# pigimonaco/Pinocchio

Hardware: AMD Instinct MI355X
Metric: grid-cells/sec for full Fmax sweep (all smoothing radii) + 3LPT, 1024^3 box (higher is better)
Workload: dtype f64

## Files before the change

### pinocchio_amd/csrc/pf_api.hip

```cpp
#include <hip/hip_runtime.h>

#include <math.h>
#include <stdarg.h>
#include <stdio.h>
#include <stdlib.h>
#include <string.h>

#include <atomic>
#include <string>
#include <functional>
#include <vector>

#include "../../include/pinfmax.h"
#include "pf_collapse_core.h"
#include "pf_hostpool.h"
#include "pf_internal.h"

extern "C" void pf_rccl_release(void *link);
extern "C" int pf_rccl_link_count(void *link);

static thread_local char g_err[512] = "";
int pf_fail(int task, const char *fmt, ...) {
  va_list ap;
  va_start(ap, fmt);
// ... 102 lines not shown
  int gt_n[4];
  double gt_logkmin[4], gt_dlogk[4], gt_sign[4];
  double *gtab;
  int tab_ns;
  double tab_var[PF_MAX_SMOOTH];
  bool tab_ready;
  int tab_ismooth;
  int model;
  double sng_cosmo[7], sng_Din[PF_MAX_SMOOTH], sng_size[PF_MAX_SMOOTH];
  int sng_ns;
  PfCtDev ct;
  double *ct_block;
  bool have_density, have_hessian, have_sources, products_init;
  int sources_order;
  bool sweep_sources, sources_fresh;
  bool transposed;
  int ct_flavour;
  int lpt_order;
  double *partials_src;
  bool general;
  void *W;
  void *fft_c2r, *fft_r2c;
  bool vel_zero_pending;
  int last_ns;
  struct PfHandoff *handoff;
  PfLoopback *loopback;
  pf_alltoall_fn a2a; void *a2a_user;
  pf_alltoallv_fn a2av; void *a2av_user;
  pf_allreduce_fn ared; void *ared_user;
  void *rccl;
// ... 107 lines not shown
  t->zpass_inv_wg_per_cu = env_int("PF_ZPASS_INV_WG_PER_CU", 32);
  if (t->zpass_inv_wg_per_cu <= 0) t->zpass_inv_wg_per_cu = 32;
  t->spline_lut = env_int("PF_SPLINE_LUT", 1) != 0;
  t->exchange_rows = env_int("PF_EXCHANGE_ROWS", 1) != 0;
  t->invariants = env_int("PF_INVARIANTS", 1);
  t->lpt_fuse = env_int("PF_LPT_FUSE", 1);
  t->collapse_wg_per_cu = env_int("PF_COLLAPSE_WG_PER_CU", 8);
  if (t->collapse_wg_per_cu <= 0) t->collapse_wg_per_cu = 8;
  t->general = env_int("PF_GENERAL", 0) != 0;

  t->pipeline = env_int("PF_PIPELINE", 1) != 0;
  t->replicate = env_int("PF_REPLICATE_DK", -1);
  t->exact_libm = env_int("PF_EXACT_LIBM", 0) != 0;
  t->solve_beside_z = env_int("PF_SOLVE_BESIDE_Z", -1);
  t->gtab = env_int("PF_GTAB", 1) != 0;
  t->preflight = env_int("PF_PREFLIGHT", 1) != 0;
  t->handoff_chunk_mb = env_int("PF_HANDOFF_CHUNK_MB", 256);
  if (t->handoff_chunk_mb <= 0) t->handoff_chunk_mb = 256;
  t->handoff_threads = env_int("PF_HANDOFF_THREADS", 0);
  t->host_register = env_int("PF_HOST_REGISTER", 0) != 0;
  t->distribute_lds = env_int("PF_DISTRIBUTE_LDS", 1) != 0;
  const char *fault = getenv("PF_DEBUG_PIPELINE_FAULT");
  t->debug_fault = !fault ? 0 : !strcmp(fault, "recv") ? 1 : !strcmp(fault, "send") ? 2 : 0;
  t->prune_eps = 8.673617379884035e-19;
  if (const char *e = getenv("PF_PRUNE_EPS")) t->prune_eps = atof(e);
}

static void plan_bytes(const pf_ctx *c, size_t *at_create, size_t *peak) {
  const size_t field = c->field_bytes, nc = ncell_of(c);
  size_t fields = 1 + 3 + 6 + 3;
// ... 131 lines not shown
  if ((cfg->flags & PF_FLAG_DOUBLE_PRODUCTS) && cfg->field_bytes != 8)
    return pf_fail(rank, "pf_create: PF_FLAG_DOUBLE_PRODUCTS (fp64 Fmax and displacements) needs fp64 fields");
  int ndev = 0;
  if (hipGetDeviceCount(&ndev) != hipSuccess || ndev <= 0)
    return pf_fail(rank, "pf_create: no HIP device available (libpinfmax_hip has no CPU path)");
  if (cfg->device < 0 || cfg->device >= ndev) return pf_fail(rank, "pf_create: device %d out of range (%d devices)", cfg->device, ndev);
  pf_ctx *c = new pf_ctx();
  c->cfg = *cfg; c->rank = rank; c->P = cfg->nranks; c->n = (int)n; c->nzh = c->n / 2 + 1; c->nzp = c->n / 2 + 64 / cfg->field_bytes;
  c->tune = tune; c->dev = cfg->device; c->inv_reruns = 0;
  c->general = want_general; c->fft_c2r = c->fft_r2c = nullptr; c->W = nullptr;
  if (c->general) c->nzp = c->nzh;
  c->nxl = c->n / c->P; c->nyl = c->n / c->P; c->fb = cfg->field_bytes; c->timing = (cfg->flags & PF_FLAG_TIMING) != 0; c->pb = (cfg->flags & PF_FLAG_DOUBLE_PRODUCTS) ? 8 : 4;
  c->dev_bytes = 0; c->own_stream = true; c->stream = nullptr;
  c->a2a = nullptr; c->a2av = nullptr; c->a2av_user = nullptr; c->ared = nullptr; c->a2a_user = c->ared_user = nullptr; c->rccl = nullptr;
  c->have_density = c->have_hessian = c->have_sources = c->products_init = false; c->last_ns = 0;
  c->sweep_sources = c->sources_fresh = false; c->partials_src = nullptr; c->lpt_order = 3; c->ct_flavour = 0; c->transposed = false;
  c->vel_zero_pending = false; c->have_genic = false;
  memset(c->ks_ms, 0, sizeof(c->ks_ms)); memset(c->ks_bytes, 0, sizeof(c->ks_bytes)); memset(c->ks_n, 0, sizeof(c->ks_n));
  memset(&c->cpu, 0, sizeof(c->cpu)); memset(c->spl_set, 0, sizeof(c->spl_set)); memset(c->spl_n, 0, sizeof(c->spl_n));
  c->growth[0] = 1.0; c->growth[1] = 3. / 7.; c->growth[2] = -1. / 9.; c->growth[3] = 5. / 42.;
  for (int i = 0; i < 6; i++) { c->B[i] = nullptr; c->B2[i] = nullptr; }
  c->blockA = nullptr; c->dk = nullptr; c->recvA = nullptr; c->tw = nullptr;
  c->blockA2 = nullptr; c->recvA2 = nullptr; c->cstream = nullptr; c->dk_full = nullptr; c->replicate = false; c->dk_full_valid = false; for (int k = 0; k < 3; k++) c->INV[0][k] = c->INV[1][k] = nullptr; c->inv_w = 0; c->inv_own[0] = c->inv_own[1] = nullptr; c->blockS = c->blockB2 = nullptr;
  c->fmax = nullptr; c->rmax = nullptr; c->vel12 = nullptr; c->partials = nullptr; c->scal = nullptr; c->hist = nullptr; c->spl = nullptr;
  c->gtab = nullptr; c->etab = nullptr; c->ct_block = nullptr; c->gt = nullptr; c->gt_lut = nullptr;
  memset(c->gt_ok, 0, sizeof(c->gt_ok)); memset(c->gt_err, 0, sizeof(c->gt_err));
  for (int i = 0; i < 2; i++) c->ev_x[i] = c->ev_r[i] = c->ev_y[i] = c->ev_s[i] = nullptr;
  c->sstream = nullptr; c->solve_ran_beside = false; c->loopback = nullptr; c->handoff = nullptr;
  c->pipeline = c->P > 1 && tune.pipeline;
  for (int i = 0; i < 3; i++) { c->A[i] = nullptr; c->S[i] = nullptr; }
  memset(c->gt_n, 0, sizeof(c->gt_n));
// ... 232 lines not shown
  PfAddr a; a.os = c->nzp; a.el_shift = ilog2i(c->n); a.el_len = c->n; a.ehs = 0; a.els = (long long)c->n * c->nzp; return a;
}
static PfAddr addr_local_x(const pf_ctx *c, int zp) {
  PfAddr a; a.os = (long long)c->nxl * zp; a.el_shift = ilog2i(c->nxl); a.el_len = c->nxl; a.ehs = 0; a.els = zp; return a;
}
static PfAddr addr_local_y(const pf_ctx *c, int zp) {
  PfAddr a; a.os = zp; a.el_shift = ilog2i(c->n); a.el_len = c->n; a.ehs = 0; a.els = (long long)c->nxl * zp; return a;
}
static PfAddr addr_xs_y(const pf_ctx *c) {
  PfAddr a; a.os = (long long)c->n * c->nzp; a.el_shift = ilog2i(c->n); a.el_len = c->n; a.ehs = 0; a.els = c->nzp; return a;
}

struct Job { const void *in; void *out; int mul; };

static int xpass(pf_ctx *c, int kind, int dir, int njobs, const Job *jobs, int pre, double rs, double growth, int nin, int band = 1 << 30,
                 bool out_yblocks = false, bool replicated = false) {
  PfStridedParams p; memset(&p, 0, sizeof(p));
  p.njobs = njobs;
  for (int j = 0; j < njobs; j++) { p.job[j].in = jobs[j].in; p.job[j].out = jobs[j].out; p.job[j].mul = jobs[j].mul; }
  p.ain = p.aout = addr_ky_x(c);
  if (out_yblocks) p.aout = addr_yblocks_x(c, band_zpitch(c, band));
  p.ncols = c->nzh; p.nouter = c->nyl; p.pre = pre; p.outer_offset = c->rank * c->nyl; p.rs = rs; p.growth = growth; p.tw = c->tw;
  p.etab = c->etab; p.dev = c->dev;
  if (replicated) {
    p.ain = addr_full_x(c); p.aout = addr_local_x(c, band_zpitch(c, band));
    p.nouter = c->n; p.outer_offset = 0; p.out_e0 = c->rank * c->nxl; p.out_ne = c->nxl;
  }
  if (pre && rs != 0.0) PFCHK(c, pf_launch_exp_table(c->etab, c->n, rs, c->stream));
  p.band_e = p.band_outer = c->n;
  double frac_cols = 1.0, frac_in = 1.0, frac_outer = 1.0;
  if (band < c->n / 2) {
    p.band_e = p.band_outer = band;
    p.ncols = band + 1;
    frac_cols = (double)(band + 1) / c->nzh; frac_in = frac_outer = (double)(2 * band + 1) / c->n;
  }
  KTimer t(c, kind, (nin * frac_in * (replicated ? c->P : 1) + njobs) * frac_cols * frac_outer * spec_bytes_alg(c));
  PFCHK(c, pf_launch_strided(c->fb, c->n, dir, p, c->stream));
  return 0;
}
static int ypass(pf_ctx *c, int kind, int dir, int njobs, const Job *jobs, bool in_blocks, bool out_blocks, int nin, int band = 1 << 30,
                 bool in_yblocks = false, bool in_local = false) {
  PfStridedParams p; memset(&p, 0, sizeof(p));
  p.njobs = njobs;
  for (int j = 0; j < njobs; j++) { p.job[j].in = jobs[j].in; p.job[j].out = jobs[j].out; p.job[j].mul = jobs[j].mul; }
  p.ain = in_blocks ? (in_yblocks ? addr_yblocks_y(c, band_zpitch(c, band)) : addr_blocks_y(c)) : addr_xs_y(c);
  if (in_local) p.ain = addr_local_y(c, band_zpitch(c, band));
  p.aout = out_blocks ? addr_blocks_y(c) : addr_xs_y(c);
  p.ncols = c->nzh; p.nouter = c->nxl; p.pre = 0; p.outer_offset = 0; p.rs = 0; p.growth = 1; p.tw = c->tw; p.dev = c->dev;
  p.band_e = p.band_outer = c->n;
  double frac_cols = 1.0, frac_in = 1.0;
  if (band < c->n / 2) {
// ... 12 lines not shown
  p.njobs = njobs;
  double outb = 0;
  for (int j = 0; j < njobs; j++) {
    p.job[j].in = jobs[j].in; p.job[j].out = jobs[j].out; p.job[j].mul = jobs[j].mul; p.job[j].out_f32 = jobs[j].f32;
    outb += jobs[j].f32 ? (double)ncell(c) * 4.0 : real_bytes_alg(c);
  }
  p.nlines = (long long)c->nxl * c->n; p.in_pitch = c->nzp; p.out_pitch = 2 * c->nzp;
  p.norm = 1.0 / ((double)c->n * c->n * c->n); p.dc = dc; p.tw = c->tw;
  p.band_k = c->n;
  double frac_in = 1.0;
  if (band < c->n / 2) { p.band_k = band; frac_in = (double)(band + 1) / c->nzh; }
  p.ncu = c->ncu; p.dev = c->dev; p.persist_per_cu = c->tune.zpass_persist; p.inv_per_cu = c->tune.zpass_inv_wg_per_cu;
  p.flag = c->scal + SC_INV_FLAG;
  if (acc) {
    p.acc = acc;
    KTimer t(c, KS_ZPASS_LPT3B, njobs * frac_in * spec_bytes_alg(c) + 8.0 * real_bytes_alg(c));
    PFCHK(c, pf_launch_c2r_invariants(c->fb, c->n, p, c->stream, 1));
    return 0;
  }
  if (invariants) {
    if (c->fb == 4) {
      if (inv_rows(c, c->inv_w)) return 1;
      for (int k = 0; k < 3; k++) p.inv_out[k] = c->INV[c->inv_w][k];
      p.inv_pitch = c->n;
      if (c->inv_w == 0) c->have_sources = false;
    }
    KTimer t(c, KS_ZPASS_INV, njobs * frac_in * spec_bytes_alg(c) + 3.0 * (double)ncell(c) * 8.0);
    PFCHK(c, pf_launch_c2r_invariants(c->fb, c->n, p, c->stream));
    return 0;
  }
  KTimer t(c, kind, njobs * frac_in * spec_bytes_alg(c) + outb);
  PFCHK(c, pf_launch_c2r(c->fb, c->n, p, c->stream));
// ... 92 lines not shown
      PFCHK(c, g_c2r(c, c->W, tmp));
      PFCHK(c, pf_launch_real_to_col((const double *)tmp, velcol(c, 3 * orders[j] + ia - 1), nc, c->pb, c->stream));
    }
  return 0;
}
static int g_forward_of(pf_ctx *c, void *f) {
  PFCHK(c, g_r2c(c, f, c->W));
  HIPCHK(c, hipMemcpyAsync(f, c->W, c->field_bytes, hipMemcpyDeviceToDevice, c->stream));
  return 0;
}
static int g_reverse_of(pf_ctx *c, void *f) {
  PFCHK(c, g_filter(c, f, c->W, -1, -1, 0.0, 0, true));
  return g_c2r(c, c->W, f);
}

static int hess_band(const pf_ctx *c, double rs) {
  int band = 1 << 30;
  if (rs > 0.0 && c->prune_eps > 0.0) {
    const double kc = sqrt(-2.0 * log(c->prune_eps)) / rs;
    const double kb = kc * c->n / (2.0 * 3.14159265358979323846);
    if (kb < c->n / 2 - 1) band = (int)kb + 1;
  }
  return band;
}
static int hess_x(pf_ctx *c, const void *spec, double rs, void *const A[3], int band, bool replicated = false) {
  const Job xj[3] = {{spec, A[0], PF_MUL_ONE}, {spec, A[1], PF_MUL_K}, {spec, A[2], PF_MUL_K2}};
  return xpass(c, KS_XPASS_HESS, +1, 3, xj, 1, rs, 1.0, 1, band, true, replicated);
}
static int ensure_dk_full(pf_ctx *c) {
  if (!c->replicate || c->dk_full_valid) return 0;
  if (c->a2a == loopback_a2a && c->have_genic) {
    unsigned int *dseed = nullptr;
    const int rc = pf_genic_launch(c->fb, c->dk_full, c->n, c->nzp, c->n, 0, &c->genic, c->stream, &dseed);
    if (!rc) HIPCHK(c, hipStreamSynchronize(c->stream));
    hipFree(dseed);
    if (rc) return pf_fail(c->rank, "pf_genic_density (whole spectrum): launch failed");
    c->dk_full_valid = true;
    return 0;
  }
  const size_t rows = (size_t)c->nyl * c->nzp * 2 * c->fb;
  HIPCHK(c, hipMemsetAsync(c->dk_full, 0, (size_t)c->P * c->field_bytes, c->stream));
  HIPCHK(c, hipMemcpy2DAsync((char *)c->dk_full + (size_t)c->rank * rows, (size_t)c->P * rows, c->dk, rows, rows, (size_t)c->n,
// ... 28 lines not shown
  return pipelined_band(c, 1, 3,
                        [&](int, void *const *A) { return hess_x(c, rep ? c->dk_full : spec, rs, A, band, rep); },
                        [&](int, int set, int f) { return recv_field(c, set, f); },
                        [&](int, const void *const *R) { return hess_yz(c, R, dc, out, band, false, acc, hfirst, rep); },
                        [&](int) { return band; }, rep);
}

static int displacements_of(pf_ctx *c, int count, const void *const *specs, const int *orders, void *const tmp[3]) {
  if (c->general) return g_displacements_of(c, count, specs, orders, tmp[0]);
  auto run = [&](int cnt, const void *const *sp, const int *ord, bool rep) -> int {
    return pipelined_band(c, cnt, 2,
                   [&](int j, void *const *A) {
                     const int o = ord[j];
                     const void *spec = rep ? c->dk_full : sp[j];
                     double growth = c->growth[o];
                     if (c->gt_n[o]) {
                       KTimer t(c, KS_MISC, 2.0 * spec_bytes_alg(c));
                       PFCHK(c, pf_launch_apply_growth(c->fb, spec, A[2], c->n, c->nyl, c->nzh, c->nzp, c->rank * c->nyl, c->gtab + o * PF_KBIN_CAP,
                                                       c->gt_n[o], c->gt_logkmin[o], c->gt_dlogk[o], c->gt_sign[o], c->stream));
                       spec = A[2];
                       growth = 1.0;
                     }
                     const Job xj[2] = {{spec, A[0], PF_MUL_ONE}, {spec, A[1], PF_MUL_IK}};
                     return xpass(c, KS_XPASS_DISP, +1, 2, xj, 1, 0.0, growth, 1, 1 << 30, true, rep);
                   },
                   [&](int, int set, int f) { return recv_field(c, set, f); },
                   [&](int j, const void *const *R) {
                     const int o = ord[j];
                     const Job yj[3] = {{R[1], tmp[0], PF_MUL_ONE}, {R[0], tmp[1], PF_MUL_IK}, {R[0], tmp[2], PF_MUL_ONE}};
                     PFCHK(c, ypass(c, KS_YPASS_DISP, +1, 3, yj, true, false, 2, 1 << 30, true, rep));
                     const int compact = c->pb == 8 ? 2 : 1;
                     const ZJob zj[3] = {{tmp[0], velcol(c, 3 * o + 0), PF_MUL_ONE, compact},
                                         {tmp[1], velcol(c, 3 * o + 1), PF_MUL_ONE, compact},
                                         {tmp[2], velcol(c, 3 * o + 2), PF_MUL_IK, compact}};
                     PFCHK(c, zpass_c2r(c, KS_ZPASS_DISP, 3, zj, nullptr));
                     return 0;
                   },
                   [](int) { return 1 << 30; }, rep);
  };
// ... 16 lines not shown
  KTimer t(c, KS_R2C_Z, real_bytes_alg(c) + spec_bytes_alg(c));
  PFCHK(c, pf_launch_r2c(c->fb, c->n, p, c->stream));
  return 0;
}
static int forward_many(pf_ctx *c, int count, void *const *fs) {
  if (c->general) {
    for (int i = 0; i < count; i++) PFCHK(c, g_forward_of(c, fs[i]));
    return 0;
  }
  if (c->P == 1) {
    for (int i = 0; i < count; i++) {
      void *f = fs[i];
      PFCHK(c, forward_r2c(c, f));
      const Job yj[1] = {{f, f, PF_MUL_ONE}};
      PFCHK(c, ypass(c, KS_YPASS_FWD, -1, 1, yj, false, false, 1));
      const Job xj[1] = {{f, f, PF_MUL_ONE}};
      PFCHK(c, xpass(c, KS_XPASS_FWD, -1, 1, xj, 0, 0.0, 1.0, 1));
    }
    return 0;
  }
  return pipelined(c, count, 1,
                   [&](int i, void *const *A) {
                     PFCHK(c, forward_r2c(c, fs[i]));
                     const Job yj[1] = {{fs[i], A[0], PF_MUL_ONE}};
                     return ypass(c, KS_YPASS_FWD, -1, 1, yj, false, true, 1);
                   },
                   [&](int i, int, int) { return fs[i]; },
                   [&](int i, const void *const *) {
                     const Job xj[1] = {{fs[i], fs[i], PF_MUL_ONE}};
                     return xpass(c, KS_XPASS_FWD, -1, 1, xj, 0, 0.0, 1.0, 1);
// ... 297 lines not shown
  }
  sources = sources && c->lpt_order >= 2 && !invariants && !c->tab_ns && !p.sng;
  size_t nb = (ncell(c) + 255) / 256;
  const size_t cap = sources ? (size_t)PF_NBLK : (size_t)c->collapse_blocks;
  if (nb > cap) nb = cap;
  p.nblocks = (int)nb;
  if (invariants) p.invariants = 1;
  int solve_fb = c->fb;
  if (invariants && c->fb == 4) {
    for (int k = 0; k < 3; k++) p.h[k] = c->INV[inv_set][k];
    p.pitch = c->n; solve_fb = 8;
  }
  if (sources) {
    p.sources = 1; p.src[0] = c->S[0]; p.src[1] = c->S[1]; p.src[2] = c->S[2]; p.src_partials = c->partials_src;
    c->have_sources = false;
  }
  {
    KTimer t(c, sources ? KS_COLLAPSE_SRC : invariants ? KS_COLLAPSE_INV : KS_COLLAPSE,
             (double)ncell(c) * ((invariants ? 3.0 * 8.0 / c->fb : sources ? 9.0 : 6.0) * c->fb + 16.0), st);
    PFCHK(c, pf_launch_collapse(solve_fb, p, st));
  }
  PFCHK(c, pf_launch_final_sum(c->partials, p.nblocks, c->scal + SC_VAR0 + 2 * ismooth, st));
  if (sources) {
    PFCHK(c, pf_launch_sum1(c->partials_src, p.nblocks, 1.0 / ((double)c->n * c->n * c->n), c->scal + SC_DC_S2, st));
    c->sources_fresh = true;
  }
  return 0;
}

static int products_reset(pf_ctx *c) {
  c->vel_zero_pending = true;
  c->products_init = true;
  return 0;
}
// ... 169 lines not shown
  if (ensure_b2(c)) return 1;
  if (!c->products_init) {
    PFCHK(c, pf_launch_fill_products(c->fmax, c->rmax, c->vel12, ncell(c), c->pb, c->stream));
    c->products_init = true;
  }
  if (recompute_sd && c->lpt_order >= 2) {
    PhaseTimer pt(c, 0);
    PFCHK(c, hessian_of(c, c->dk, 0.0, c->scal + SC_DC_DK, c->B));
    c->have_hessian = true; c->sources_fresh = false;
  }
  {
    PhaseTimer pt(c, 2);
    if (compute_sources && c->lpt_order >= 2) {
      if (!c->have_hessian) return pf_fail(c->rank, "pf_displacements: second derivatives at R=0 not in place");
      if (!c->sources_fresh) {
      PfLptSrcParams sp; memset(&sp, 0, sizeof(sp));
      for (int i = 0; i < 6; i++) sp.h[i] = c->B[i];
      sp.s2 = c->S[0]; sp.s3a = c->S[1]; sp.s3b = c->S[2]; sp.pitch = rpitch(c); sp.nrows = (long long)c->nxl * c->n; sp.n = c->n;
      sp.partials = c->partials;
      size_t nb = (ncell(c) + 255) / 256; if (nb > PF_NBLK) nb = PF_NBLK;
      sp.nblocks = (int)nb;
      {
        KTimer t(c, KS_LPT_SRC, 9.0 * real_bytes_alg(c));
        PFCHK(c, pf_launch_lpt_sources(c->fb, sp, c->stream));
      }
      PFCHK(c, pf_launch_sum1(c->partials, sp.nblocks, 1.0 / ((double)c->n * c->n * c->n), c->scal + SC_DC_S2, c->stream));
      }
      c->sources_fresh = false;
      PFCHK(c, allreduce_dev(c, c->scal + SC_DC_S2, 1, 0));
      PFCHK(c, forward_of(c, c->S[0]));
      const bool fuse3b = (c->tune.lpt_fuse >= 2 ? pf_c2r_invariants_supported(c->fb, (int)c->n) : pf_c2r_invariants_preferred(c->fb, (int)c->n)) && !c->general && c->tune.lpt_fuse;
      if (c->lpt_order < 3) {
      } else if (fuse3b) {
        PFCHK(c, hessian_of(c, c->S[0], 0.0, c->scal + SC_DC_S2, c->B2, c->S[2], c->B));
      } else {
        PFCHK(c, hessian_of(c, c->S[0], 0.0, c->scal + SC_DC_S2, c->B2));
        PfLptAccParams ap; memset(&ap, 0, sizeof(ap));
        for (int i = 0; i < 6; i++) { ap.h[i] = c->B[i]; ap.phi2[i] = c->B2[i]; }
        ap.s3b = c->S[2]; ap.pitch = rpitch(c); ap.nrows = (long long)c->nxl * c->n; ap.n = c->n;
        KTimer t(c, KS_LPT_ACC, 14.0 * real_bytes_alg(c));
        PFCHK(c, pf_launch_lpt_accum(c->fb, ap, c->stream));
      }
      void *const s12[2] = {c->S[1], c->S[2]};
      if (c->lpt_order >= 3) PFCHK(c, forward_many(c, 2, s12));
      c->have_sources = true; c->sources_order = c->lpt_order;
    } else if (c->lpt_order >= 2 && (!c->have_sources || c->sources_order < c->lpt_order))
// ... 483 lines not shown
  };
  return handoff_d2h(c, (char *)host, nullptr, nc * rec, rec, fill);
}

extern "C" int pf_get_second_derivative(pf_ctx *c, int i, double *host) {
  if (!c || !host || i < 0 || i > 5) return pf_fail(0, "pf_get_second_derivative: bad argument");
  if (!c->have_hessian) return pf_fail(c->rank, "pf_get_second_derivative: not computed");
  const long long nrows = (long long)c->nxl * c->n;
  PFCHK(c, pf_launch_real_export(c->fb, c->B[i], (double *)staging(c), nrows, c->n, rpitch(c), c->stream));
  return handoff_d2h(c, (char *)host, staging(c), (size_t)nrows * c->n * sizeof(double), 1, no_fill);
}

extern "C" int pf_get_kvector(pf_ctx *c, int which, double *host) {
  if (!c || !host || which < 0 || which > 2) return pf_fail(0, "pf_get_kvector: bad argument");
  if (!c->have_sources) return pf_fail(c->rank, "pf_get_kvector: LPT sources not computed");
  return export_spec(c, c->S[which], host);
}
extern "C" int pf_debug_replicated_rows(pf_ctx *c, int kx0, int nkx, double *host) {
  if (!c || !host || kx0 < 0 || nkx < 1 || kx0 + nkx > c->n) return pf_fail(0, "pf_debug_replicated_rows: bad argument");
  if (!c->replicate) return pf_fail(c->rank, "pf_debug_replicated_rows: this context does not keep the whole spectrum (PF_REPLICATE_DK)");
  if (!c->have_density) return pf_fail(c->rank, "pf_debug_replicated_rows: density not set");
  PFCHK(c, ensure_dk_full(c));
  const long long nrows = (long long)nkx * c->n;
  if ((size_t)nrows * c->nzh * 2 * sizeof(double) > 2 * c->field_bytes) return pf_fail(c->rank, "pf_debug_replicated_rows: %d rows exceed the staging area", nkx);
  const char *src = (const char *)c->dk_full + (size_t)kx0 * c->n * c->nzp * 2 * c->fb;
  PFCHK(c, pf_launch_spec_export(c->fb, src, (double *)staging(c), nrows, c->nzh, c->nzp, c->stream));
  return handoff_d2h(c, (char *)host, staging(c), (size_t)nrows * c->nzh * 2 * sizeof(double), 1, no_fill);
}
extern "C" int pf_get_density(pf_ctx *c, double *host) {
  if (!c || !host) return 1;
// ... 372 lines not shown
```

### pinocchio_amd/csrc/pf_cell_kernels.hip

```cpp
#include <type_traits>

#include "pf_internal.h"
#include "pf_fft_core.h"
#include "pf_collapse_core.h"
#include "pf_sng_core.h"

#define PF_CELL_BLOCK 256
#ifndef PF_SOLVE_INV_BLOCK
#define PF_SOLVE_INV_BLOCK 512
#endif
#ifndef PF_SOLVE_INV_WAVES
#define PF_SOLVE_INV_WAVES 4
#endif
#define PF_MAX_KNOTS 512
#ifndef PF_C3_TABLE
#define PF_C3_TABLE 1
#endif

__device__ __forceinline__ void pf_block_sum2(double &a, double &b, double *sh ) {
#pragma unroll
  for (int off = 32; off > 0; off >>= 1) {
    a += __shfl_down(a, off, 64);
    b += __shfl_down(b, off, 64);
  }
// ... 10 lines not shown
#pragma unroll
  for (int off = 32; off > 0; off >>= 1) {
    a += __shfl_down(a, off, 64);
    b += __shfl_down(b, off, 64);
  }
  const int lane = threadIdx.x & 63, w = threadIdx.x >> 6;
  if (lane == 0) { sh[2 * w] = a; sh[2 * w + 1] = b; }
  __syncthreads();
  if (threadIdx.x % 256 == 0) {
    double sa = 0, sb = 0;
    for (int i = w; i < w + 4; i++) { sa += sh[2 * i]; sb += sh[2 * i + 1]; }
    a = sa; b = sb;
  }
}

PF_HD void pf_lpt_sources_cell(const double d[6], double &src2, double &src31, double &src32) {
  src2 = d[0] * d[1] + d[0] * d[2] + d[1] * d[2] - d[3] * d[3] - d[4] * d[4] - d[5] * d[5];
  src31 = 3.0 * (d[0] * (d[1] * d[2] - d[5] * d[5]) - d[3] * (d[3] * d[2] - d[4] * d[5]) + d[4] * (d[3] * d[5] - d[4] * d[1]));
  src32 = 2.0 * (d[0] + d[1] + d[2]) * src2;
}
template <typename F, bool FAST, bool TAB = false, bool INV = false, bool SNG = false, bool SRC = false, int FLAV = 0, typename PR = float>
__device__ __forceinline__ void pf_collapse_body(const PfCollapseParams &p) {
  constexpr bool GT = FAST && !TAB && !SNG;
  constexpr int SK = TAB ? PF_CT_NBINS_D : GT ? (PF_GT_MAX_INT + 1) * PF_GT_REC : 5 * PF_MAX_KNOTS;
  static_assert(!GT || SK >= 5 * PF_MAX_KNOTS, "the knot arrays fit the table's place");
  __shared__ double sk[SK];
  __shared__ double red[2 * ((PF_SOLVE_INV_BLOCK > PF_CELL_BLOCK ? PF_SOLVE_INV_BLOCK : PF_CELL_BLOCK) / 64)];
  __shared__ unsigned short slut[TAB ? 1 : GT ? PF_GT_MAX_BINS : PF_SPLINE_LUT_BINS];
  constexpr bool C3 = FAST && !SNG && PF_C3_TABLE;
  __shared__ double sc3[C3 ? PF_C3_DOUBLES : 1];
  if (C3) for (int i = threadIdx.x; i < PF_C3_DOUBLES; i += blockDim.x) sc3[i] = pf_c3_tab[i];
  const int nk = p.spline.n;
  const bool gt = GT && p.spline.gt != nullptr;
  pf_spline_view sv;
  if (gt) {
// ... 90 lines not shown
    double d[6];
#pragma unroll
    for (int k = 0; k < 6; k++) d[k] = dn[k];
    const PR fold = foldn;
    const long long a = an;
    row += srow; col += scol;
    if (PF_SOLVE_PREFETCH && i + stride < ncell) {
      if (col >= p.n) { col -= p.n; row++; }
      fetch(i + stride, (long long)row * p.pitch + col);
    }
    if (SRC) {
      double src2, src31, src32;
      pf_lpt_sources_cell(d, src2, src31, src32);
      s2[a] = (F)src2;
      s3a[a] = (F)src31;
      s3b[a] = (F)src32;
      sum_src += (double)(F)src2;
    }
    const double delta = INV ? d[0] : d[0] + d[1] + d[2];
    sum += delta;
    sum2 += delta * delta;
    double lam[3];
    bool have_lam;
    if (INV) {
      const double third = d[0] * (1.0 / 3.0);
      const double diag[3] = {third, third, third};
      have_lam = pf_eigen_from_invariants<FAST>(d[0], d[1], d[2], diag, lam, c3tab);
    } else {
      have_lam = pf_ordered_eigenvalues<FAST>(d, lam, c3tab);
    }
    const double Fnew = !have_lam ? -10.0
// ... 694 lines not shown
```

### pinocchio_amd/csrc/pf_collapse_core.h

```cpp
#pragma once
#include <math.h>
#include "pf_gtab.h"
#include "pf_c3tab.h"

#if defined(__clang__)
#pragma clang fp contract(off)
#endif

#ifndef PF_HD
#if defined(__HIPCC__)
#define PF_HD __host__ __device__ __forceinline__
#else
#define PF_HD inline
#endif
#endif

#define PF_PI 3.14159265358979323846
#define PF_SMALL 1.e-20

struct pf_spline_view {
  const double *x, *y, *c, *b, *d;
  int n;
  const unsigned short *lut = nullptr;
  double lut_inv_w = 0.0, lut_x0 = 0.0;
// ... 344 lines not shown
    const double inv_del = FAST ? pf_div_fast(1.0, del) : 1.0 / del;
    const double arg = -6.5 * (l1 - l2) * inv_del - 2.8 * (l2 - l3) * inv_del;
    ell += -.364 * inv_del * (FAST ? pf_exp_series(arg) : exp(arg));
  }
  return ell;
}
template <bool FAST = false> PF_HD double pf_ell_classic(double l1, double l2, double l3, const double *c3tab = nullptr) {
  double ell = 0.0;
  pf_cubic c;
  const int kind = pf_ell_setup<FAST>(l1, l2, l3, ell, c);
  if (kind == 1) ell = pf_ell_one_root<FAST>(c);
  else if (kind == 2) ell = pf_ell_three_roots<FAST>(c, c3tab);
  return pf_ell_finish<FAST>(ell, l1, l2, l3);
}

PF_HD double pf_lpt3b_accumulate(double s, const double phi2[6], const double h[6]) {
#if defined(__clang__)
#pragma clang fp contract(off)
#endif
  const int order[6] = {0, 3, 4, 1, 5, 2};
#if defined(__HIP_DEVICE_COMPILE__)
#pragma unroll
#endif
  for (int j = 0; j < 6; j++) {
    const int c = order[j];
    const double f = 2.0 * (c < 3 ? 1.0 : 2.0);
    s -= f * phi2[c] * h[c];
  }
  return s;
}
// ... 340 lines not shown
```

### pinocchio_amd/csrc/pf_fft_kernels.hip

```cpp
#include <atomic>
#include <cstdio>

#include "pf_internal.h"
#include "pf_fft_core.h"

#include "pf_fft_stages.h"
#include "pf_fft16.h"
#include "pf_strided_addr.h"
#include "pf_collapse_core.h"

#ifndef PF_SLAB_STORE
#define PF_SLAB_STORE 1
#endif
template <typename F> struct PfCols {
  using S = F;
  static constexpr int n = 1;
  static __device__ __forceinline__ pfc<F> load(const pfc<S> *base, long long off) { return pf_ld_stream(base + off); }
  static __device__ __forceinline__ void store(pfc<S> *base, long long off, pfc<F> v, bool) { pf_st_stream(base + off, v); }
  static __device__ __forceinline__ pfc<F> load_ul(const pfc<S> *base, long long u, unsigned lane) {
    return pf_ld_stream(reinterpret_cast<const pfc<S> *>(reinterpret_cast<const char *>(base + u) + (size_t)(lane * (unsigned)sizeof(pfc<S>))));
  }
  static __device__ __forceinline__ void store_ul(pfc<S> *base, long long u, unsigned lane, pfc<F> v, bool) {
    pf_st_stream(reinterpret_cast<pfc<S> *>(reinterpret_cast<char *>(base + u) + (size_t)(lane * (unsigned)sizeof(pfc<S>))), v);
  }
// ... 20 lines not shown
#else
      *reinterpret_cast<f4 *>(base + off) = t;
#endif
    } else {
      pf_st_stream(base + off, pf_mk<float>(v.x.x, v.y.x));
    }
  }
  static __device__ __forceinline__ pfc<pf_f32x2> load_ul(const pfc<float> *base, long long u, unsigned lane) {
    return load(reinterpret_cast<const pfc<float> *>(reinterpret_cast<const char *>(base + u) + (size_t)(lane * (unsigned)sizeof(pfc<float>))), 0);
  }
  static __device__ __forceinline__ void store_ul(pfc<float> *base, long long u, unsigned lane, pfc<pf_f32x2> v, bool v1) {
    store(reinterpret_cast<pfc<float> *>(reinterpret_cast<char *>(base + u) + (size_t)(lane * (unsigned)sizeof(pfc<float>))), 0, v, v1);
  }
};

template <typename F, int N, int T, int DIR, bool FA>
__global__ void __launch_bounds__(T *N / 8) __attribute__((amdgpu_waves_per_eu(4))) k_strided(const PfStridedParams p, const long long nwork, const int ntiles) {
  using C = pfc<F>;
  using COLS = PfCols<F>;
  using S = typename COLS::S;
  constexpr int NL = COLS::n;
  constexpr int NT = N / 8;
#ifndef PF_PAIR16
#define PF_PAIR16 1
#endif
  constexpr bool P16 = PF_PAIR16 && pf_pair16_length(N) && T == 8;
  extern __shared__ __attribute__((aligned(16))) char smem[];
  C *lds = reinterpret_cast<C *>(smem);
  const long long w = pf_xcd_swizzle(blockIdx.x, (nwork + 7) >> 3);
  if (w >= nwork) return;
  const int tid = threadIdx.x;
  const int c = tid % T, tl = tid / T;
// ... 11 lines not shown

  C src[8], v[8];
  auto load_tile = [&](const void *inp, int tlj, int colj) {
    const pfc<S> *__restrict__ in = reinterpret_cast<const pfc<S> *>(inp);
#pragma unroll
    for (int m = 0; m < 8; m++) {
      const int e = pf_line_index<N, P16>(tlj, m);
      const int se = e > N / 2 ? e - N : e;
      const bool inband = se <= p.band_e && se >= -p.band_e;
      if constexpr (FA) src[m] = (valid && inband) ? COLS::load_ul(in, pf_addr_uniform<NT>(p.ain, outer, m, NL * tile * T), pf_addr_lane(p.ain, pf_line_index<N, P16>(tlj, 0), colj - NL * tile * T)) : pf_zero<F>();
      else src[m] = (valid && inband) ? COLS::load(in, pf_addr(p.ain, outer, e, colj)) : pf_zero<F>();
      if constexpr (NL > 1) { if (!valid1) { src[m].x.y = 0.f; src[m].y.y = 0.f; } }
    }
  };
  load_tile(p.job[0].in, tl, col);
  double ko = 0.0, woc[NL];
#pragma unroll
  for (int l = 0; l < NL; l++) woc[l] = 1.0;
  if (p.pre) {
    int so = outer + p.outer_offset;
    if (so > N / 2) so -= N;
    ko = kf * so;
#pragma unroll
    for (int l = 0; l < NL; l++) {
      const double kc = kf * (col + l);
      const double ko2kc2 = ko * ko + kc * kc;
      woc[l] = (p.rs != 0.0 ? exp(-0.5 * ko2kc2 * p.rs * p.rs) : 1.0) * p.growth;
    }
  }
#pragma unroll 1
// ... 322 lines not shown
        __builtin_nontemporal_store(w2, reinterpret_cast<pf_d2 *>(o2 + ao));
        __builtin_nontemporal_store(w3, reinterpret_cast<pf_d2 *>(o3 + ao));
#else
        *reinterpret_cast<double2 *>(o1 + ao) = make_double2(a1, b1);
        *reinterpret_cast<double2 *>(o2 + ao) = make_double2(a2, b2);
        *reinterpret_cast<double2 *>(o3 + ao) = make_double2(a3, b3);
#endif
      } else {
        double ha[6], hb[6];
#pragma unroll
        for (int k = 0; k < 6; k++) {
          const F2 g = *reinterpret_cast<const F2 *>(reinterpret_cast<const F *>(p.job[k].out) + a);
          ha[k] = (double)g.x; hb[k] = (double)g.y;
        }
        F2 *acc = reinterpret_cast<F2 *>(reinterpret_cast<F *>(p.acc) + a);
        const F2 s = *acc;
        F2 r;
        r.x = (F)pf_lpt3b_accumulate((double)s.x, da, ha);
        r.y = (F)pf_lpt3b_accumulate((double)s.y, db, hb);
        *acc = r;
      }
    }
  };
  if (SPEC && reducer) {
    constexpr int LINE_BARRIERS = NT > 64 ? 3 + 2 * (pf_nstages(M) - 1) : 0;
#pragma unroll 1
    for (long long Rr = blockIdx.x; Rr < nrows; Rr += gridDim.x) {
      int tr = tid - TL * NT;
      asm volatile("" : "+v"(tr));
#pragma unroll
      for (int i = 0; i < LINE_BARRIERS; i++) __syncthreads();
// ... 374 lines not shown
  return launch_strided_v<F, N, DIR, false>(p, st, ntiles, nwork);
}
#ifndef PF_F32_PAIRS
#define PF_F32_PAIRS 1
#endif
template <int N, int DIR>
static int launch_strided_f32(const PfStridedParams &p, hipStream_t st) {
  if constexpr (N == 2048 || N == 1024) {
    const int rc = pf_launch_strided16(4, N, DIR, p, st);
    if (rc >= 0) return rc;
  }
  if constexpr (PF_F32_PAIRS && N >= 1024) return launch_strided_n<pf_f32x2, N, DIR>(p, st);
  else return launch_strided_n<float, N, DIR>(p, st);
}

template <typename F, int N>
static int launch_c2r_n(const PfC2RParams &p, hipStream_t st) {
  constexpr int M = N / 2, NT = M / 8;
  constexpr int TL = (NT >= 256) ? 1 : 256 / NT;
  constexpr int LPL = (M + 1 > M + M / 8) ? M + 1 : M + M / 8;
  const long long nblk = (p.nlines + TL - 1) / TL;
  dim3 grid((unsigned)(nblk * p.njobs), 1, 1), block(TL * NT, 1, 1);
  const size_t shm = (size_t)TL * LPL * sizeof(pfc<F>);
  const int persist = p.persist_per_cu;
  if (persist > 0 && N >= 64 && p.ncu > 0) {
    const long long ntiles = nblk * p.njobs;
    long long g = (long long)p.ncu * persist;
    if (g > ntiles) g = ntiles;
    hipLaunchKernelGGL((k_c2r_persistent<F, N, TL>), dim3((unsigned)g), block, shm, st, p, ntiles);
    return hipGetLastError() == hipSuccess ? 0 : 1;
  }
  hipLaunchKernelGGL((k_c2r<F, N, TL>), grid, block, shm, st, p);
  return hipGetLastError() == hipSuccess ? 0 : 1;
}

template <typename F, int N>
static int launch_c2r_invariants_n(const PfC2RParams &p, hipStream_t st, int mode) {
  constexpr int M = N / 2, NT = M / 8;
  constexpr int LPL = PfZiPlan<F, M>::line;
  long long g = (long long)(p.ncu > 0 ? p.ncu : 256) * (p.inv_per_cu > 0 ? p.inv_per_cu : 32);
  if (g > p.nlines) g = p.nlines;
  const size_t shm = (size_t)6 * LPL * sizeof(pfc<F>);
  if (mode == 1) {
    if constexpr (PfZiPlan<F, M>::spec(1)) hipLaunchKernelGGL((k_c2r_invariants_spec<F, N, 1>), dim3((unsigned)g), dim3(6 * NT + 64 * PfZiPlan<F, M>::reducer_waves), shm, st, p, p.nlines);
    else hipLaunchKernelGGL((k_c2r_invariants<F, N, 1>), dim3((unsigned)g), dim3(6 * NT), shm, st, p, p.nlines);
  } else if constexpr (PF_ZI_PK2 && sizeof(F) == 4 && N >= 512 && N <= PF_ZI_PK2_MAXN) {
    for (int j = 0; j < 6; j++) if (p.job[j].mul == PF_MUL_IK) return 2;
    constexpr int RW = N >= 2048 ? 4 : (N >= 1024 ? 2 : 1);
    constexpr int LPL2 = M + M / 16 + 1;
    const size_t shm2 = (size_t)6 * LPL2 * sizeof(PfRow2);
    const int threads = 6 * NT + 64 * RW;
    static std::atomic<bool> raised2[PF_MAX_DEVICES];
    if (shm2 > 64 * 1024 && p.dev >= 0 && p.dev < PF_MAX_DEVICES && !raised2[p.dev].load(std::memory_order_acquire)) {
      if (hipFuncSetAttribute(reinterpret_cast<const void *>(&k_c2r_invariants_pk2<N, RW>), hipFuncAttributeMaxDynamicSharedMemorySize, (int)shm2) != hipSuccess) return 3;
      raised2[p.dev].store(true, std::memory_order_release);
    }
    long long g2 = g;
    const long long npairs = (p.nlines + 1) / 2;
    if (g2 > npairs) g2 = npairs;
    hipLaunchKernelGGL((k_c2r_invariants_pk2<N, RW>), dim3((unsigned)g2), dim3(threads), shm2, st, p, p.nlines);
// ... 40 lines not shown
#undef CALL
    }
  } else {
    if (dir > 0) {
#define CALL(NN) launch_strided_f32<NN, +1>(p, st)
      PF_SWITCH_N(n, CALL)
#undef CALL
    } else {
#define CALL(NN) launch_strided_f32<NN, -1>(p, st)
      PF_SWITCH_N(n, CALL)
#undef CALL
    }
  }
}

int pf_launch_c2r(int fb, int n, const PfC2RParams &p, hipStream_t st) {
  if (n & (n - 1)) return pf_launch_mixed_c2r(fb, n, p, st);
  if (fb == 8) {
#define CALL(NN) launch_c2r_n<double, NN>(p, st)
    PF_SWITCH_N(n, CALL)
#undef CALL
  } else {
#define CALL(NN) launch_c2r_n<float, NN>(p, st)
    PF_SWITCH_N(n, CALL)
#undef CALL
  }
}

bool pf_c2r_invariants_supported(int fb, int n) {
  if (n & (n - 1)) return pf_mixed_invariants_supported(fb, n);
  return n >= 16 && n <= (fb == 8 ? 1024 : 2048);
}
bool pf_c2r_invariants_preferred(int fb, int n) {
  return pf_c2r_invariants_supported(fb, n) && (!(n & (n - 1)) || (fb == 8 && pf_mixed_plan_compiled_in(n)));
}
int pf_launch_c2r_invariants(int fb, int n, const PfC2RParams &p, hipStream_t st, int mode) {
  if (p.njobs != 6 || (mode == 1 && !p.acc) || (mode == 0 && !p.flag) || !pf_c2r_invariants_supported(fb, n)) return 2;
  if (fb == 4 && mode == 0 && (!p.inv_out[0] || !p.inv_out[1] || !p.inv_out[2])) return 2;
  if (n & (n - 1)) return pf_launch_mixed_c2r_invariants(fb, n, p, st, mode);
  if (fb == 8) {
#define CALL(NN) launch_c2r_invariants_n<double, NN>(p, st, mode)
    PF_SWITCH_N(n, CALL)
#undef CALL
  } else {
    if (mode == 0 && (!p.inv_out[0] || !p.inv_out[1] || !p.inv_out[2])) return 2;
#define CALL(NN) launch_c2r_invariants_n<float, NN>(p, st, mode)
    PF_SWITCH_N(n, CALL)
#undef CALL
  }
}

int pf_launch_r2c(int fb, int n, const PfR2CParams &p, hipStream_t st) {
  if (n & (n - 1)) return pf_launch_mixed_r2c(fb, n, p, st);
  if (fb == 8) {
// ... 10 lines not shown
```

### pinocchio_amd/csrc/pf_internal.h

```cpp
#pragma once
#include <hip/hip_runtime.h>
#include <stddef.h>
#include <stdint.h>

#include "../../include/pinfmax.h"

#define PF_MAX_JOBS 6
#define PF_MAX_DEVICES 64

struct PfTuning {
  int zpass_persist;
  int zpass_inv_wg_per_cu;
  int collapse_wg_per_cu;
  bool spline_lut, exchange_rows, general, pipeline, exact_libm;
  int invariants, lpt_fuse;
  int replicate;
  double prune_eps;
  int debug_fault;
  int solve_beside_z;
  int handoff_chunk_mb, handoff_threads;
  bool host_register;
  bool preflight;
  bool distribute_lds;
  bool gtab;
};

enum { PF_MUL_ONE = 0, PF_MUL_K = 1, PF_MUL_K2 = 2, PF_MUL_IK = 3 };

struct PfAddr {
  long long os;
  int el_shift;
  long long ehs, els;
  int el_len;
};

struct PfStridedJob {
  const void *in;
  void *out;
  int mul;
// ... 4 lines not shown
  PfStridedJob job[PF_MAX_JOBS];
  PfAddr ain, aout;
  int ncols;
  int nouter;
  int pre;
  int outer_offset;
  double rs, growth;
  const double *etab;
  const void *tw;
  int band_e, band_outer;
  int dev;
  int out_e0, out_ne;
};

int pf_launch_strided(int field_bytes, int n, int dir, const PfStridedParams &p, hipStream_t st);
int pf_launch_exp_table(double *etab, int n, double rs, hipStream_t st);
int pf_launch_strided16(int field_bytes, int n, int dir, const PfStridedParams &p, hipStream_t st);

struct PfC2RJob {
  const void *in;
  void *out;
  int mul;
  int out_f32;
};

struct PfC2RParams {
  int njobs;
  PfC2RJob job[PF_MAX_JOBS];
  long long nlines;
  long long in_pitch;
// ... 213 lines not shown
```

Measured before the change: 1.496 billion.

## Fuse deferred forward x-FFT into inverse x-pass and recompute 3LPT(b) start in z-pass

The forward x-transform of the LPT source spectra is now deferred and folded into the following inverse strided x-pass, which first runs the forward stages on the loaded tile. This avoids a separate full read/write of each source spectrum. The 3LPT(b) start value is no longer written by the collapse kernel when possible. The z-pass invariants kernel recomputes it from the Hessian in a new mode 2, saving one field store and load. Both add state tracking and fallbacks that finish the pending transform when the fused path cannot apply.

```diff
diff --git a/pinocchio_amd/csrc/pf_api.hip b/pinocchio_amd/csrc/pf_api.hip
--- a/pinocchio_amd/csrc/pf_api.hip
+++ b/pinocchio_amd/csrc/pf_api.hip
@@ -140,6 +140,8 @@
   bool have_density, have_hessian, have_sources, products_init;
   int sources_order;
   bool sweep_sources, sources_fresh;
+  bool x_pending[3];
+  bool s3b_start_absent;
   bool transposed;
   int ct_flavour;
   int lpt_order;
@@ -277,6 +279,8 @@
   t->exact_libm = env_int("PF_EXACT_LIBM", 0) != 0;
   t->solve_beside_z = env_int("PF_SOLVE_BESIDE_Z", -1);
   t->gtab = env_int("PF_GTAB", 1) != 0;
+  t->lpt_xfuse = env_int("PF_LPT_XFUSE", 1) != 0;
+  t->lpt3b_start = env_int("PF_LPT3B_START", 0) != 0;
   t->preflight = env_int("PF_PREFLIGHT", 1) != 0;
   t->handoff_chunk_mb = env_int("PF_HANDOFF_CHUNK_MB", 256);
   if (t->handoff_chunk_mb <= 0) t->handoff_chunk_mb = 256;
@@ -438,7 +442,7 @@
   c->dev_bytes = 0; c->own_stream = true; c->stream = nullptr;
   c->a2a = nullptr; c->a2av = nullptr; c->a2av_user = nullptr; c->ared = nullptr; c->a2a_user = c->ared_user = nullptr; c->rccl = nullptr;
   c->have_density = c->have_hessian = c->have_sources = c->products_init = false; c->last_ns = 0;
-  c->sweep_sources = c->sources_fresh = false; c->partials_src = nullptr; c->lpt_order = 3; c->ct_flavour = 0; c->transposed = false;
+  c->sweep_sources = c->sources_fresh = false; c->x_pending[0] = c->x_pending[1] = c->x_pending[2] = false; c->s3b_start_absent = false; c->partials_src = nullptr; c->lpt_order = 3; c->ct_flavour = 0; c->transposed = false;
   c->vel_zero_pending = false; c->have_genic = false;
   memset(c->ks_ms, 0, sizeof(c->ks_ms)); memset(c->ks_bytes, 0, sizeof(c->ks_bytes)); memset(c->ks_n, 0, sizeof(c->ks_n));
   memset(&c->cpu, 0, sizeof(c->cpu)); memset(c->spl_set, 0, sizeof(c->spl_set)); memset(c->spl_n, 0, sizeof(c->spl_n));
@@ -701,7 +705,7 @@
 struct Job { const void *in; void *out; int mul; };
 
 static int xpass(pf_ctx *c, int kind, int dir, int njobs, const Job *jobs, int pre, double rs, double growth, int nin, int band = 1 << 30,
-                 bool out_yblocks = false, bool replicated = false) {
+                 bool out_yblocks = false, bool replicated = false, bool fwd_first = false) {
   PfStridedParams p; memset(&p, 0, sizeof(p));
   p.njobs = njobs;
   for (int j = 0; j < njobs; j++) { p.job[j].in = jobs[j].in; p.job[j].out = jobs[j].out; p.job[j].mul = jobs[j].mul; }
@@ -722,6 +726,11 @@
     frac_cols = (double)(band + 1) / c->nzh; frac_in = frac_outer = (double)(2 * band + 1) / c->n;
   }
   KTimer t(c, kind, (nin * frac_in * (replicated ? c->P : 1) + njobs) * frac_cols * frac_outer * spec_bytes_alg(c));
+  if (fwd_first) {
+    if (dir < 0 || replicated) return pf_fail(c->rank, "xpass: a pending forward x-transform goes with an inverse pass over this rank's own spectrum");
+    PFCHK(c, pf_launch_strided_xfuse(c->fb, c->n, p, c->stream));
+    return 0;
+  }
   PFCHK(c, pf_launch_strided(c->fb, c->n, dir, p, c->stream));
   return 0;
 }
@@ -764,8 +773,10 @@
   p.flag = c->scal + SC_INV_FLAG;
   if (acc) {
     p.acc = acc;
-    KTimer t(c, KS_ZPASS_LPT3B, njobs * frac_in * spec_bytes_alg(c) + 8.0 * real_bytes_alg(c));
-    PFCHK(c, pf_launch_c2r_invariants(c->fb, c->n, p, c->stream, 1));
+    const bool start_here = c->s3b_start_absent;
+    KTimer t(c, KS_ZPASS_LPT3B, njobs * frac_in * spec_bytes_alg(c) + (start_here ? 7.0 : 8.0) * real_bytes_alg(c));
+    PFCHK(c, pf_launch_c2r_invariants(c->fb, c->n, p, c->stream, start_here ? 2 : 1));
+    c->s3b_start_absent = false;
     return 0;
   }
   if (invariants) {
@@ -888,6 +899,13 @@
   return g_c2r(c, c->W, f);
 }
 
+static bool lpt3b_in_zpass(const pf_ctx *c) {
+  return (c->tune.lpt_fuse >= 2 ? pf_c2r_invariants_supported(c->fb, (int)c->n) : pf_c2r_invariants_preferred(c->fb, (int)c->n)) && !c->general && c->tune.lpt_fuse;
+}
+static bool lpt3b_start_in_zpass(const pf_ctx *c) {
+  return lpt3b_in_zpass(c) && !c->tune.lpt3b_start && c->sweep_sources && c->lpt_order >= 3 && c->P == 1 && !(c->n & (c->n - 1));
+}
+
 static int hess_band(const pf_ctx *c, double rs) {
   int band = 1 << 30;
   if (rs > 0.0 && c->prune_eps > 0.0) {
@@ -897,9 +915,21 @@
   }
   return band;
 }
+static int x_pending_of(const pf_ctx *c, const void *spec) {
+  for (int i = 0; i < 3; i++) if (c->x_pending[i] && spec == c->S[i]) return i;
+  return -1;
+}
+static int finish_forward_x(pf_ctx *c, int i) {
+  const Job xj[1] = {{c->S[i], c->S[i], PF_MUL_ONE}};
+  PFCHK(c, xpass(c, KS_XPASS_FWD, -1, 1, xj, 0, 0.0, 1.0, 1));
+  c->x_pending[i] = false;
+  return 0;
+}
 static int hess_x(pf_ctx *c, const void *spec, double rs, void *const A[3], int band, bool replicated = false) {
   const Job xj[3] = {{spec, A[0], PF_MUL_ONE}, {spec, A[1], PF_MUL_K}, {spec, A[2], PF_MUL_K2}};
-  return xpass(c, KS_XPASS_HESS, +1, 3, xj, 1, rs, 1.0, 1, band, true, replicated);
+  int pend = replicated ? -1 : x_pending_of(c, spec);
+  if (pend >= 0 && band < c->n / 2) { PFCHK(c, finish_forward_x(c, pend)); pend = -1; }
+  return xpass(c, KS_XPASS_HESS, +1, 3, xj, 1, rs, 1.0, 1, band, true, replicated, pend >= 0);
 }
 static int ensure_dk_full(pf_ctx *c) {
   if (!c->replicate || c->dk_full_valid) return 0;
@@ -958,6 +988,8 @@
                      const int o = ord[j];
                      const void *spec = rep ? c->dk_full : sp[j];
                      double growth = c->growth[o];
+                     int pend = rep ? -1 : x_pending_of(c, spec);
+                     if (pend >= 0 && c->gt_n[o]) { PFCHK(c, finish_forward_x(c, pend)); pend = -1; }
                      if (c->gt_n[o]) {
                        KTimer t(c, KS_MISC, 2.0 * spec_bytes_alg(c));
                        PFCHK(c, pf_launch_apply_growth(c->fb, spec, A[2], c->n, c->nyl, c->nzh, c->nzp, c->rank * c->nyl, c->gtab + o * PF_KBIN_CAP,
@@ -966,7 +998,7 @@
                        growth = 1.0;
                      }
                      const Job xj[2] = {{spec, A[0], PF_MUL_ONE}, {spec, A[1], PF_MUL_IK}};
-                     return xpass(c, KS_XPASS_DISP, +1, 2, xj, 1, 0.0, growth, 1, 1 << 30, true, rep);
+                     return xpass(c, KS_XPASS_DISP, +1, 2, xj, 1, 0.0, growth, 1, 1 << 30, true, rep, pend >= 0);
                    },
                    [&](int, int set, int f) { return recv_field(c, set, f); },
                    [&](int j, const void *const *R) {
@@ -1013,6 +1045,10 @@
       PFCHK(c, forward_r2c(c, f));
       const Job yj[1] = {{f, f, PF_MUL_ONE}};
       PFCHK(c, ypass(c, KS_YPASS_FWD, -1, 1, yj, false, false, 1));
+      int si = -1;
+      for (int k = 0; k < 3; k++) if (f == c->S[k]) si = k;
+      if (si >= 0) c->x_pending[si] = c->tune.lpt_xfuse && pf_strided_xfuse_supported(c->fb, (int)c->n);
+      if (si >= 0 && c->x_pending[si]) continue;
       const Job xj[1] = {{f, f, PF_MUL_ONE}};
       PFCHK(c, xpass(c, KS_XPASS_FWD, -1, 1, xj, 0, 0.0, 1.0, 1));
     }
@@ -1340,10 +1376,12 @@
   if (sources) {
     p.sources = 1; p.src[0] = c->S[0]; p.src[1] = c->S[1]; p.src[2] = c->S[2]; p.src_partials = c->partials_src;
     c->have_sources = false;
+    c->s3b_start_absent = lpt3b_start_in_zpass(c);
+    if (c->s3b_start_absent) p.src[2] = nullptr;
   }
   {
     KTimer t(c, sources ? KS_COLLAPSE_SRC : invariants ? KS_COLLAPSE_INV : KS_COLLAPSE,
-             (double)ncell(c) * ((invariants ? 3.0 * 8.0 / c->fb : sources ? 9.0 : 6.0) * c->fb + 16.0), st);
+             (double)ncell(c) * ((invariants ? 3.0 * 8.0 / c->fb : sources ? (p.src[2] ? 9.0 : 8.0) : 6.0) * c->fb + 16.0), st);
     PFCHK(c, pf_launch_collapse(solve_fb, p, st));
   }
   PFCHK(c, pf_launch_final_sum(c->partials, p.nblocks, c->scal + SC_VAR0 + 2 * ismooth, st));
@@ -1543,6 +1581,7 @@
     if (compute_sources && c->lpt_order >= 2) {
       if (!c->have_hessian) return pf_fail(c->rank, "pf_displacements: second derivatives at R=0 not in place");
       if (!c->sources_fresh) {
+      c->s3b_start_absent = false;
       PfLptSrcParams sp; memset(&sp, 0, sizeof(sp));
       for (int i = 0; i < 6; i++) sp.h[i] = c->B[i];
       sp.s2 = c->S[0]; sp.s3a = c->S[1]; sp.s3b = c->S[2]; sp.pitch = rpitch(c); sp.nrows = (long long)c->nxl * c->n; sp.n = c->n;
@@ -1558,7 +1597,9 @@
       c->sources_fresh = false;
       PFCHK(c, allreduce_dev(c, c->scal + SC_DC_S2, 1, 0));
       PFCHK(c, forward_of(c, c->S[0]));
-      const bool fuse3b = (c->tune.lpt_fuse >= 2 ? pf_c2r_invariants_supported(c->fb, (int)c->n) : pf_c2r_invariants_preferred(c->fb, (int)c->n)) && !c->general && c->tune.lpt_fuse;
+      const bool fuse3b = lpt3b_in_zpass(c);
+      if (c->lpt_order < 3) c->s3b_start_absent = false;
+      if (c->s3b_start_absent && !fuse3b) return pf_fail(c->rank, "pf_displacements: the sweep left the 3LPT(b) start value to a z-pass that does not run");
       if (c->lpt_order < 3) {
       } else if (fuse3b) {
         PFCHK(c, hessian_of(c, c->S[0], 0.0, c->scal + SC_DC_S2, c->B2, c->S[2], c->B));
@@ -2072,6 +2113,7 @@
 extern "C" int pf_get_kvector(pf_ctx *c, int which, double *host) {
   if (!c || !host || which < 0 || which > 2) return pf_fail(0, "pf_get_kvector: bad argument");
   if (!c->have_sources) return pf_fail(c->rank, "pf_get_kvector: LPT sources not computed");
+  if (c->x_pending[which]) PFCHK(c, finish_forward_x(c, which));
   return export_spec(c, c->S[which], host);
 }
 extern "C" int pf_debug_replicated_rows(pf_ctx *c, int kx0, int nkx, double *host) {
diff --git a/pinocchio_amd/csrc/pf_cell_kernels.hip b/pinocchio_amd/csrc/pf_cell_kernels.hip
--- a/pinocchio_amd/csrc/pf_cell_kernels.hip
+++ b/pinocchio_amd/csrc/pf_cell_kernels.hip
@@ -48,11 +48,6 @@
   }
 }
 
-PF_HD void pf_lpt_sources_cell(const double d[6], double &src2, double &src31, double &src32) {
-  src2 = d[0] * d[1] + d[0] * d[2] + d[1] * d[2] - d[3] * d[3] - d[4] * d[4] - d[5] * d[5];
-  src31 = 3.0 * (d[0] * (d[1] * d[2] - d[5] * d[5]) - d[3] * (d[3] * d[2] - d[4] * d[5]) + d[4] * (d[3] * d[5] - d[4] * d[1]));
-  src32 = 2.0 * (d[0] + d[1] + d[2]) * src2;
-}
 template <typename F, bool FAST, bool TAB = false, bool INV = false, bool SNG = false, bool SRC = false, int FLAV = 0, typename PR = float>
 __device__ __forceinline__ void pf_collapse_body(const PfCollapseParams &p) {
   constexpr bool GT = FAST && !TAB && !SNG;
@@ -173,7 +168,7 @@
       pf_lpt_sources_cell(d, src2, src31, src32);
       s2[a] = (F)src2;
       s3a[a] = (F)src31;
-      s3b[a] = (F)src32;
+      if (s3b) s3b[a] = (F)src32;
       sum_src += (double)(F)src2;
     }
     const double delta = INV ? d[0] : d[0] + d[1] + d[2];
diff --git a/pinocchio_amd/csrc/pf_collapse_core.h b/pinocchio_amd/csrc/pf_collapse_core.h
--- a/pinocchio_amd/csrc/pf_collapse_core.h
+++ b/pinocchio_amd/csrc/pf_collapse_core.h
@@ -382,6 +382,14 @@
   return pf_ell_finish<FAST>(ell, l1, l2, l3);
 }
 
+PF_HD void pf_lpt_sources_cell(const double d[6], double &src2, double &src31, double &src32) {
+#if defined(__clang__)
+#pragma clang fp contract(off)
+#endif
+  src2 = d[0] * d[1] + d[0] * d[2] + d[1] * d[2] - d[3] * d[3] - d[4] * d[4] - d[5] * d[5];
+  src31 = 3.0 * (d[0] * (d[1] * d[2] - d[5] * d[5]) - d[3] * (d[3] * d[2] - d[4] * d[5]) + d[4] * (d[3] * d[5] - d[4] * d[1]));
+  src32 = 2.0 * (d[0] + d[1] + d[2]) * src2;
+}
 PF_HD double pf_lpt3b_accumulate(double s, const double phi2[6], const double h[6]) {
 #if defined(__clang__)
 #pragma clang fp contract(off)
diff --git a/pinocchio_amd/csrc/pf_fft_kernels.hip b/pinocchio_amd/csrc/pf_fft_kernels.hip
--- a/pinocchio_amd/csrc/pf_fft_kernels.hip
+++ b/pinocchio_amd/csrc/pf_fft_kernels.hip
@@ -58,8 +58,11 @@
   }
 };
 
-template <typename F, int N, int T, int DIR, bool FA>
+constexpr int PF_DIR_XF = 2;
+template <typename F, int N, int T, int DIRS, bool FA>
 __global__ void __launch_bounds__(T *N / 8) __attribute__((amdgpu_waves_per_eu(4))) k_strided(const PfStridedParams p, const long long nwork, const int ntiles) {
+  constexpr bool XF = DIRS == PF_DIR_XF;
+  constexpr int DIR = XF ? +1 : DIRS;
   using C = pfc<F>;
   using COLS = PfCols<F>;
   using S = typename COLS::S;
@@ -101,6 +104,18 @@
     }
   };
   load_tile(p.job[0].in, tl, col);
+  if constexpr (XF) {
+    PfStages<F, N, -1, 1, 0, false, P16>::run(
+        src, tl, tw, [&](int pos, C val) { lds[pos * T + c] = val; }, [&](int pos) { return lds[pos * T + c]; });
+    if constexpr (P16) {
+#pragma unroll
+      for (int m = 0; m < 8; m++) lds[(tl + m * NT) * T + c] = src[m];
+      __syncthreads();
+#pragma unroll
+      for (int m = 0; m < 8; m++) src[m] = lds[pf_line_index<N, P16>(tl, m) * T + c];
+      __syncthreads();
+    }
+  }
   double ko = 0.0, woc[NL];
 #pragma unroll
   for (int l = 0; l < NL; l++) woc[l] = 1.0;
@@ -453,7 +468,13 @@
           ha[k] = (double)g.x; hb[k] = (double)g.y;
         }
         F2 *acc = reinterpret_cast<F2 *>(reinterpret_cast<F *>(p.acc) + a);
-        const F2 s = *acc;
+        F2 s;
+        if constexpr (MODE == 2) {
+          double s2, s31, sa, sb;
+          pf_lpt_sources_cell(ha, s2, s31, sa);
+          pf_lpt_sources_cell(hb, s2, s31, sb);
+          s.x = (F)sa; s.y = (F)sb;
+        } else s = *acc;
         F2 r;
         r.x = (F)pf_lpt3b_accumulate((double)s.x, da, ha);
         r.y = (F)pf_lpt3b_accumulate((double)s.y, db, hb);
@@ -858,6 +879,12 @@
   else return launch_strided_n<float, N, DIR>(p, st);
 }
 
+template <int N>
+static int launch_strided_xf_f32(const PfStridedParams &p, hipStream_t st) {
+  if constexpr (N < 1024) return launch_strided_n<float, N, PF_DIR_XF>(p, st);
+  else return 2;
+}
+
 template <typename F, int N>
 static int launch_c2r_n(const PfC2RParams &p, hipStream_t st) {
   constexpr int M = N / 2, NT = M / 8;
@@ -888,6 +915,9 @@
   if (mode == 1) {
     if constexpr (PfZiPlan<F, M>::spec(1)) hipLaunchKernelGGL((k_c2r_invariants_spec<F, N, 1>), dim3((unsigned)g), dim3(6 * NT + 64 * PfZiPlan<F, M>::reducer_waves), shm, st, p, p.nlines);
     else hipLaunchKernelGGL((k_c2r_invariants<F, N, 1>), dim3((unsigned)g), dim3(6 * NT), shm, st, p, p.nlines);
+  } else if (mode == 2) {
+    if constexpr (PfZiPlan<F, M>::spec(1)) hipLaunchKernelGGL((k_c2r_invariants_spec<F, N, 2>), dim3((unsigned)g), dim3(6 * NT + 64 * PfZiPlan<F, M>::reducer_waves), shm, st, p, p.nlines);
+    else hipLaunchKernelGGL((k_c2r_invariants<F, N, 2>), dim3((unsigned)g), dim3(6 * NT), shm, st, p, p.nlines);
   } else if constexpr (PF_ZI_PK2 && sizeof(F) == 4 && N >= 512 && N <= PF_ZI_PK2_MAXN) {
     for (int j = 0; j < 6; j++) if (p.job[j].mul == PF_MUL_IK) return 2;
     constexpr int RW = N >= 2048 ? 4 : (N >= 1024 ? 2 : 1);
@@ -958,6 +988,22 @@
   }
 }
 
+bool pf_strided_xfuse_supported(int fb, int n) { return !(n & (n - 1)) && n >= 16 && n <= 2048 && (fb == 8 || n < 1024); }
+int pf_launch_strided_xfuse(int fb, int n, const PfStridedParams &p, hipStream_t st) {
+  if (!pf_strided_xfuse_supported(fb, n) || p.njobs < 1 || p.band_e < n / 2 || p.band_outer < n / 2 || p.out_ne > 0) return 2;
+  for (int j = 1; j < p.njobs; j++) if (p.job[j].in != p.job[0].in) return 2;
+  for (int j = 0; j < p.njobs; j++) if (p.job[j].out == p.job[0].in) return 2;
+  if (fb == 8) {
+#define CALL(NN) launch_strided_n<double, NN, PF_DIR_XF>(p, st)
+    PF_SWITCH_N(n, CALL)
+#undef CALL
+  } else {
+#define CALL(NN) launch_strided_xf_f32<NN>(p, st)
+    PF_SWITCH_N(n, CALL)
+#undef CALL
+  }
+}
+
 int pf_launch_c2r(int fb, int n, const PfC2RParams &p, hipStream_t st) {
   if (n & (n - 1)) return pf_launch_mixed_c2r(fb, n, p, st);
   if (fb == 8) {
@@ -979,9 +1025,9 @@
   return pf_c2r_invariants_supported(fb, n) && (!(n & (n - 1)) || (fb == 8 && pf_mixed_plan_compiled_in(n)));
 }
 int pf_launch_c2r_invariants(int fb, int n, const PfC2RParams &p, hipStream_t st, int mode) {
-  if (p.njobs != 6 || (mode == 1 && !p.acc) || (mode == 0 && !p.flag) || !pf_c2r_invariants_supported(fb, n)) return 2;
+  if (p.njobs != 6 || (mode >= 1 && !p.acc) || (mode == 0 && !p.flag) || mode < 0 || mode > 2 || !pf_c2r_invariants_supported(fb, n)) return 2;
   if (fb == 4 && mode == 0 && (!p.inv_out[0] || !p.inv_out[1] || !p.inv_out[2])) return 2;
-  if (n & (n - 1)) return pf_launch_mixed_c2r_invariants(fb, n, p, st, mode);
+  if (n & (n - 1)) return mode == 2 ? 2 : pf_launch_mixed_c2r_invariants(fb, n, p, st, mode);
   if (fb == 8) {
 #define CALL(NN) launch_c2r_invariants_n<double, NN>(p, st, mode)
     PF_SWITCH_N(n, CALL)
diff --git a/pinocchio_amd/csrc/pf_internal.h b/pinocchio_amd/csrc/pf_internal.h
--- a/pinocchio_amd/csrc/pf_internal.h
+++ b/pinocchio_amd/csrc/pf_internal.h
@@ -23,6 +23,8 @@
   bool preflight;
   bool distribute_lds;
   bool gtab;
+  bool lpt3b_start;
+  bool lpt_xfuse;
 };
 
 enum { PF_MUL_ONE = 0, PF_MUL_K = 1, PF_MUL_K2 = 2, PF_MUL_IK = 3 };
@@ -57,6 +59,8 @@
 };
 
 int pf_launch_strided(int field_bytes, int n, int dir, const PfStridedParams &p, hipStream_t st);
+bool pf_strided_xfuse_supported(int field_bytes, int n);
+int pf_launch_strided_xfuse(int field_bytes, int n, const PfStridedParams &p, hipStream_t st);
 int pf_launch_exp_table(double *etab, int n, double rs, hipStream_t st);
 int pf_launch_strided16(int field_bytes, int n, int dir, const PfStridedParams &p, hipStream_t st);
 
```

Result: faster. 1.514 billion (median of 6 runs) (+1.2%).
